# furiosa-ai/eta-inversion

Hardware: AMD Instinct MI355X
Metric: images/sec SD1.5 512^2 50-step etainv+ptp (higher is better)
Workload: dtype bf16; 1 GPU; etainv+ptp, SD1.5-shaped UNet (seeded synthetic weights), 512x512 (64x64 latents), 50 DDIM steps, 32 image pairs per GPU per step, eta [[0.6, 0], [1, 0.7]], n=10 noise candidates, cfg 7.5/1; images_per_gpu=32, unet_sample_forwards_per_image_reference=300

## Files before the change

eta-inversion_amd/csrc/engine.cpp:

```cpp
#include <cmath>
#include <cstring>
#include <functional>
#include <memory>
#include <string>
#include <unordered_map>
#include <vector>

#include "common.h"
#include "kernels.h"

namespace etainv {

static thread_local std::string g_err;
void set_error(const std::string& msg) { g_err = msg; }

struct ProfRec { int cls; double work, bytes; hipEvent_t a, b; };
static bool g_prof_on = false;
static std::vector<ProfRec> g_prof;
static std::vector<std::pair<hipEvent_t, hipEvent_t>> g_prof_pool;
static size_t g_prof_used = 0;
static bool g_prof_paused = false;
bool prof_enabled() { return g_prof_on && !g_prof_paused; }
void prof_pause(bool on) { g_prof_paused = on; }
void prof_begin(int cls, double work, hipStream_t s, double bytes) {
// ... 1380 lines not shown
  p.W = wd;
  p.Ho = upsample ? h * 2 : (stride == 2 ? h / 2 : h);
  p.Wo = upsample ? wd * 2 : (stride == 2 ? wd / 2 : wd);
  p.stride = stride;
  p.ups = upsample;
  p.taps = taps;
  p.M = b * p.Ho * p.Wo;
  p.N = cout;
  p.rows_per_batch = p.Ho * p.Wo;
  return launch_igemm(p, dtype, (hipStream_t)stream);
}

extern "C" int etainv_op_gemm_f32out(const void* a, const void* w, const float* bias, float* out_f32, int m, int n, int k, int dtype, void* stream) {
  IGemmParams p;
  p.a1 = a;
  p.w = w;
  p.bias = bias;
  p.out = out_f32;
  p.out_f32 = 1;
  p.M = m;
  p.N = n;
  p.c1 = k;
  p.W = m;
  p.Wo = m;
  p.rows_per_batch = m;
  return launch_igemm(p, dtype, (hipStream_t)stream);
}

extern "C" int etainv_op_gn_fold(const float* w, const float* gamma, const float* beta, const float* bias, const float* stats, int groups, int b, int n,
                                 int k, void* wb_out, float* cb_out, int dtype, void* stream) {
  return launch_gn_fold(w, gamma, beta, bias, stats, groups, b, n, k, wb_out, cb_out, dtype, (hipStream_t)stream);
}

extern "C" int etainv_op_gemm_per_image(const void* a, const void* wb, const float* cb, const void* residual, void* out, int b, int hw, int n, int k,
                                        int dtype, void* stream) {
  ETAINV_CHECK(b > 0 && hw > 0, "bad sizes");
  IGemmParams p;
  p.a1 = a;
  p.w = wb;
  p.bias = cb;
  p.residual = residual;
  p.out = out;
  p.M = b * hw;
  p.N = n;
  p.c1 = k;
  p.W = p.M;
  p.Wo = p.M;
  p.rows_per_batch = hw;
  p.w_batch_stride = (int64_t)n * k;
  p.bias_batch_stride = n;
  return launch_igemm(p, dtype, (hipStream_t)stream);
}

extern "C" int etainv_op_time_embedding(const int64_t* t_host, int rows, int dim, void* out, int dtype, int via_device, float* t_dev, void* stream) {
  if (!via_device) return launch_time_embedding(t_host, rows, dim, out, dtype, (hipStream_t)stream);
  ETAINV_CHECK(t_dev, "via_device needs t_dev");
  if (launch_set_timesteps(t_host, rows, t_dev, (hipStream_t)stream)) return 1;
  return launch_time_embedding_dev(t_dev, rows, dim, out, dtype, (hipStream_t)stream);
}

extern "C" int etainv_op_silu(const void* x, void* out, int64_t n, int dtype, void* stream) {
  ETAINV_CHECK(x && out && n >= 0, "null pointer or negative size");
  if (n == 0) return 0;
  return launch_silu(x, out, n, dtype, (hipStream_t)stream);
}

extern "C" int etainv_op_cast(const void* src, int src_dtype, void* dst, int dst_dtype, int64_t n, void* stream) {
  ETAINV_CHECK(src && dst && n >= 0, "null pointer or negative size");
  if (n == 0) return 0;
  return launch_cast_f32(src, src_dtype, dst, dst_dtype, n, (hipStream_t)stream);
}

extern "C" int etainv_op_im2col_in(const void* latent, int io_dtype, int n_lat, int rows, int l, void* out, int dtype, void* stream) {
  ETAINV_CHECK(l > 0, "bad sizes");
  return launch_im2col_in(latent, io_dtype, n_lat, rows, l, out, dtype, (hipStream_t)stream);
}

extern "C" int etainv_op_pack_weight(const float* src, void* dst, int64_t rows, int64_t cols, int mode, int taps, float scale, const float* colscale,
                                     int dtype, void* stream) {
  return launch_pack_weight(src, dst, rows, cols, mode, taps, dtype, (hipStream_t)stream, scale, colscale);
}

extern "C" int etainv_op_word_maps_ex(const float* maps_acc, int n_layers, int n_img_cap, int heads, int res, int L, int n_img, const int32_t* tokens,
                                      int n_tok, int steps_done, int row_sel, unsigned layer_mask, float* out, int accumulate, float scale, void* stream) {
  ETAINV_CHECK(row_sel == 0 || row_sel == 1, "row_sel: 0 = source cond row, 1 = target cond row");
  ETAINV_CHECK(n_img <= n_img_cap && heads > 0 && res > 0 && L > 0, "bad sizes");
  return launch_word_maps(maps_acc, n_layers, n_img_cap, 2, row_sel, heads, res, L, n_img, tokens, n_tok, steps_done, out, accumulate, scale,
                          (hipStream_t)stream, layer_mask);
}

extern "C" int etainv_op_word_maps(const float* maps_acc, int n_layers, int n_img_cap, int heads, int res, int L, int n_img,
                                   const int32_t* tokens, int n_tok, int steps_done, float* out, int accumulate, float scale,
                                   void* stream) {
  return launch_word_maps(maps_acc, n_layers, n_img_cap, 2, 0, heads, res, L, n_img, tokens, n_tok, steps_done, out, accumulate, scale,
                          (hipStream_t)stream);
}

extern "C" int etainv_op_local_blend(const float* maps_acc, int n_layers, int n_img_cap, int heads, int res, int L, float* x, int n_img,
                                     const float* blend_alpha, float thres, void* stream) {
  return launch_local_blend(maps_acc, n_layers, n_img_cap, heads, res, L, x, n_img, blend_alpha, thres, (hipStream_t)stream);
}
```

eta-inversion_amd/csrc/igemm.hip:

```cpp
#include <cstdio>
#include <cstdlib>
#include <vector>
#include <type_traits>

#include "common.h"
#include "kernels.h"

namespace etainv {

template <typename T> struct Mfma;
template <> struct Mfma<f16> {
  typedef f16x8 frag;
  static __device__ __forceinline__ f32x4 run(frag a, frag b, f32x4 c) { return __builtin_amdgcn_mfma_f32_16x16x32_f16(a, b, c, 0, 0, 0); }
};
template <> struct Mfma<bf16> {
  typedef bf16x8 frag;
  static __device__ __forceinline__ f32x4 run(frag a, frag b, f32x4 c) { return __builtin_amdgcn_mfma_f32_16x16x32_bf16(a, b, c, 0, 0, 0); }
};

constexpr int BK = 64;
constexpr int64_t SPLITK_WS_BYTES = 64ll << 20;


__device__ __forceinline__ void chan_merge_equal(float n, float& mean, float& m2, float mb, float m2b) {
// ... 1141 lines not shown
  return 0;
#endif
  p.xcd_gn = STAGES == 3 ? pick_xcd_gn(p, BM, BN, grid, tiles) : 1;
  ProfScope prof(PROF_IGEMM, 2.0 * (double)p.M * (double)p.N * (double)(p.taps * (p.c1 + p.c2)), s, igemm_algo_bytes(p));
  hipLaunchKernelGGL((igemm_kernel<T, BM, BN, WAVES_M, STAGES, UPS, LN, PATCH>), dim3(grid), dim3(WAVES_M * 128), lds, s, p);
  ETAINV_LAUNCH_CHECK();
  return 0;
}

template <typename T>
__global__ void __launch_bounds__(256) splitk_reduce_kernel(IGemmParams p) {
  const int n4 = p.N >> 2;
  const int64_t total = (int64_t)p.M * n4;
  for (int64_t idx = (int64_t)blockIdx.x * 256 + threadIdx.x; idx < total; idx += (int64_t)gridDim.x * 256) {
    const int m = (int)(idx / n4), n = (int)(idx - (int64_t)m * n4) * 4;
    f32x4 v = *reinterpret_cast<const f32x4*>(p.ws + (int64_t)m * p.N + n);
    for (int k = 1; k < p.ksplit; ++k) v += *reinterpret_cast<const f32x4*>(p.ws + ((int64_t)k * p.M + m) * p.N + n);
    if (p.ln_stat) {
      v = (v - p.ln_stat[(int64_t)m * 2] * *reinterpret_cast<const f32x4*>(p.ln_s + n)) * p.ln_stat[(int64_t)m * 2 + 1];
    }
    if (p.bias) v += *reinterpret_cast<const f32x4*>(p.bias + (int64_t)(m / p.rows_per_batch) * p.bias_batch_stride + n);
    if (p.rowvec) v += *reinterpret_cast<const f32x4*>(p.rowvec + (int64_t)(m / p.rows_per_batch) * p.rowvec_stride + n);
    if (p.residual) {
      const T* r = reinterpret_cast<const T*>(p.residual) + (int64_t)m * p.N + n;
      v[0] += to_f32(r[0]); v[1] += to_f32(r[1]); v[2] += to_f32(r[2]); v[3] += to_f32(r[3]);
    }
    T o[4] = {from_f32<T>(v[0]), from_f32<T>(v[1]), from_f32<T>(v[2]), from_f32<T>(v[3])};
    *reinterpret_cast<u32x2*>(reinterpret_cast<T*>(p.out) + (int64_t)m * p.N + n) = *reinterpret_cast<u32x2*>(o);
  }
}

static int ring_min_tiles() {
  static const int v = env_int("ETAINV_RING_MIN_TILES", 144);
  return v;
}
static bool ring_fills(const IGemmParams& p) { return (int64_t)cdiv(p.M, 256) * cdiv(p.N, 160) >= ring_min_tiles() && !env_on("ETAINV_NO_RING"); }
static bool ln_ring_ok(const IGemmParams& p) { return !p.ln_stat || p.rows_per_batch % 64 == 0; }

bool igemm_ups4_ok(const IGemmParams& p, int dtype) {
  if (dtype == ETAINV_F32 || p.taps != 4 || p.stride != 1 || p.a2 || p.geglu || p.residual || p.rowvec || p.ln_stat || p.out_f32 || p.out_nchw || p.w_batch_stride || p.pad0) return false;
  if (p.N % 160 != 0 || p.Ho != 2 * p.H || p.Wo != 2 * p.W || p.M % (4 * p.H * p.W) != 0 || p.rows_per_batch != 4 * p.H * p.W) return false;
  if ((p.H * p.W) % 256 != 0 && ((p.M >> 2) % 256 != 0 || (p.H * p.W) % 64 != 0 || !env_flag("ETAINV_UPS4_PM", true))) return false;
  if (p.stat_out && p.stat_kind != 1) return false;
  return env_flag("ETAINV_UPS4", true) && ring_fills(p);
}

bool igemm_hm_ok(const IGemmParams& p, int dtype) {
  if (dtype == ETAINV_F32 || !p.hm_heads || !p.ln_stat || p.geglu || p.taps != 1 || p.a2 || p.residual || p.stat_out || p.out_f32 || p.out_nchw || p.w_batch_stride) return false;
  if ((p.hm_dim != 40 && p.hm_dim != 80) || p.hm_heads != 8 || p.hm_tokens > 16384 || p.M >= (1 << 24)) return false;
  if (p.N != 3 * p.hm_heads * p.hm_dim || p.N % 160 != 0 || p.hm_tokens % 256 != 0 || p.M % p.hm_tokens != 0 || !ln_ring_ok(p)) return false;
  return ring_fills(p);
}

enum IGemmRoute { ROUTE_PPCONV, ROUTE_DUALN, ROUTE_RING_UPS4, ROUTE_RING_UPS9, ROUTE_RING_PATCH, ROUTE_RING, ROUTE_RING_GEGLU, ROUTE_TWO_SLOT };
static const char* const kIGemmRouteName[] = {"ppconv", "dualn", "ring-ups4", "ring-ups9", "ring-patch", "ring", "ring-geglu", "two-slot"};

static IGemmRoute igemm_route(const IGemmParams& p, int dtype) {
  if (pp_conv_applicable(p, dtype)) return ROUTE_PPCONV;
  if (pp_dualn_applicable(p, dtype)) return ROUTE_DUALN;
  if (!p.geglu && p.ups == 2) return ROUTE_RING_UPS4;
  if (!p.geglu && p.ups == 1 && p.N % 160 == 0 && ring_fills(p)) return ROUTE_RING_UPS9;
  if (!p.geglu && p.taps == 9 && p.stride == 1 && !p.ups && !p.a2 && !p.pad0 && p.H % 16 == 0 && p.W % 16 == 0 && p.H == p.Ho && p.W == p.Wo &&
      p.N % 160 == 0 && !p.ln_stat && !p.out_nchw && !p.out_f32 && !p.w_batch_stride && (!p.stat_out || p.stat_kind == 1) &&
      env_flag("ETAINV_PATCHCONV", true) && ring_fills(p))
    return ROUTE_RING_PATCH;
  if (!p.geglu && !p.ups && p.N % 160 == 0 && ring_fills(p) && ln_ring_ok(p)) return ROUTE_RING;
  if (p.geglu && ln_ring_ok(p) && p.c1 >= env_int("ETAINV_GEGLU_RING_MINK", 320) && (int64_t)cdiv(p.M, 256) * cdiv(p.N, 128) >= 256 && !env_on("ETAINV_NO_RING"))
    return ROUTE_RING_GEGLU;
  return ROUTE_TWO_SLOT;
}

static int launch_two_slot(const IGemmParams& p, int dtype, hipStream_t s, int* stat_P) {
  const int64_t big_tiles = (int64_t)cdiv(p.M, 128) * cdiv(p.N, 128);
  static const int deepk_min_tiles = env_int("ETAINV_DEEPK_MIN_TILES", 64);
  static const int deepk_min_nk = env_int("ETAINV_DEEPK_MIN_NK", 64);
  const bool deep_k = !p.geglu && p.N % 160 == 0 && p.taps * (p.c1 + p.c2) / BK >= deepk_min_nk && !p.out_nchw && !p.out_f32 &&
                      (int64_t)cdiv(p.M, 128) * cdiv(p.N, 160) >= deepk_min_tiles;
  const bool big = p.geglu || (big_tiles >= 192 && p.N > 64) || deep_k;
  const int cfg = (big && !p.geglu && p.N % 160 == 0) ? 0 : big ? 1 : 2;
  const int bm = cfg == 2 ? 64 : 128, bn = cfg == 0 ? 160 : cfg == 1 ? 128 : 64;
  const int slots = cfg == 2 ? 1024 : 512;
  const int64_t tiles = (int64_t)cdiv(p.M, bm) * cdiv(p.N, bn);
  const int nk = p.taps * (p.c1 + p.c2) / BK;
  int ks = 1;
  if (!p.geglu && !p.out_nchw && !p.out_f32 && tiles * 2 <= slots && nk >= 16 && !env_on("ETAINV_NO_SPLITK")) {
    static const int max_split = env_int("ETAINV_SPLITK_MAX", 32);
    for (int d = 2; d <= max_split; ++d)
      if (nk % d == 0 && nk / d >= 4 && tiles * d <= slots && (int64_t)p.M * p.N * d * 4 <= SPLITK_WS_BYTES) ks = d;
  }
  static const bool trace = env_on("ETAINV_TRACE_IGEMM");
  if (trace) fprintf(stderr, "  two-slot tile=%dx%d ksplit=%d\n", bm, bn, ks);
  IGemmParams pk = p;
  if (ks > 1) {
    static float* ws[kMaxDevices] = {};
    const int dev = current_device();
    if (!ws[dev]) ETAINV_HIP(hipMalloc(&ws[dev], SPLITK_WS_BYTES));
    pk.ksplit = ks;
    pk.ws = ws[dev];
    pk.bias = nullptr;
    pk.rowvec = nullptr;
    pk.residual = nullptr;
    pk.ln_stat = nullptr;
    pk.stat_out = nullptr;
  }
  ProfScope prof(PROF_IGEMM, 2.0 * (double)p.M * (double)p.N * (double)(p.taps * (p.c1 + p.c2)), s, igemm_algo_bytes(p));
  prof_pause(true);
  int rc = 0;
  ETAINV_DISPATCH_HALF(dtype, T, rc = cfg == 0   ? launch_igemm_t<T, 128, 160, 2, 2, 0, 0>(pk, s, stat_P)
                                      : cfg == 1 ? launch_igemm_t<T, 128, 128, 2, 2, 0, 0>(pk, s, stat_P)
                                                 : launch_igemm_t<T, 64, 64, 2, 2, 0, 0>(pk, s, stat_P));
  prof_pause(false);
// ... 2 lines not shown
    IGemmParams pr = p;
    pr.ksplit = ks;
    pr.ws = pk.ws;
    const int64_t total = (int64_t)p.M * (p.N >> 2);
    ETAINV_DISPATCH_HALF(dtype, T, hipLaunchKernelGGL(splitk_reduce_kernel<T>, dim3((unsigned)std::min<int64_t>(cdiv(total, 256), 2048)),
                                                      dim3(256), 0, s, pr));
    ETAINV_LAUNCH_CHECK();
  }
  return 0;
}

int launch_igemm(const IGemmParams& p_in, int dtype, hipStream_t s, int* stat_P) {
  if (stat_P) *stat_P = 0;
  if (dtype == ETAINV_F32) return launch_igemm_f32(p_in, s);
  static void* zero_pages[kMaxDevices] = {};
  const int dev = current_device();
  if (!zero_pages[dev]) {
    ETAINV_HIP(hipMalloc(&zero_pages[dev], 256));
    ETAINV_HIP(hipMemset(zero_pages[dev], 0, 256));
  }
  IGemmParams p = p_in;
  p.zeros = zero_pages[dev];
  p.debug = env_int("ETAINV_IGEMM_DEBUG", p.debug);
  ETAINV_CHECK(p.a1 && p.w && p.out, "null pointer");
  ETAINV_CHECK(p.M > 0 && p.N > 0 && (p.N % 4) == 0, "N must be a positive multiple of 4");
  ETAINV_CHECK(p.c1 % BK == 0 && p.c2 % BK == 0 && (p.c1 + p.c2) > 0, "channel counts must be multiples of 64");
  ETAINV_CHECK(p.taps == 1 || p.taps == 9 || (p.taps == 4 && p.ups == 2), "taps must be 1 or 9 (4: the phase form of a fused-upsample conv, ups == 2)");
  ETAINV_CHECK(p.taps != 1 || (p.stride == 1 && !p.ups), "1x1 / Linear: stride 1, no upsample");
  ETAINV_CHECK(p.ups != 2 || igemm_ups4_ok(p, dtype), "phase form of the fused-upsample conv: not available for this launch (ask igemm_ups4_ok first)");
  ETAINV_CHECK(!p.geglu || (p.N % 128) == 0, "GEGLU needs N % 128 == 0");
  ETAINV_CHECK(p.rows_per_batch > 0, "rows_per_batch");
  ETAINV_CHECK(!p.rowvec || p.rowvec_stride >= p.N, "rowvec_stride");
  ETAINV_CHECK(!p.ln_stat || (p.ln_s && p.bias && p.taps == 1 && !p.a2), "folded LayerNorm: s / c vectors, plain GEMM");
  ETAINV_CHECK(!p.ln_stat || (!p.residual && !p.rowvec && !p.stat_out), "folded LayerNorm: no residual / row vector / statistics output on the consumer");
  ETAINV_CHECK(!p.ln_stat || (!p.out_f32 && !p.out_nchw), "folded LayerNorm: the consumer stores the compute dtype, row-major (the fp32 / NCHW epilogues do not apply mean / rstd)");
  ETAINV_CHECK(!p.hm_heads || igemm_hm_ok(p, dtype), "head-major QKV output: not available for this launch (ask igemm_hm_ok first)");
  ETAINV_CHECK(!p.out_nchw || p.N == 4, "out_nchw needs N == 4");
  if (p.hm_heads) p.hm_magic = (int)(((1ull << 38) + (unsigned)p.hm_tokens - 1) / (unsigned)p.hm_tokens);
  const IGemmRoute route = igemm_route(p, dtype);
  static const bool trace = env_on("ETAINV_TRACE_IGEMM");
  if (trace)
    fprintf(stderr, "igemm M=%d N=%d c1=%d c2=%d taps=%d stride=%d ups=%d H=%d W=%d geglu=%d ln=%d stat=%d res=%d rowvec=%d hm=%d route=%s\n", p.M, p.N, p.c1, p.c2, p.taps,
            p.stride, p.ups, p.H, p.W, (int)p.geglu, p.ln_stat ? 1 : 0, p.stat_out ? p.stat_kind : 0, p.residual ? 1 : 0, p.rowvec ? 1 : 0, p.hm_heads,
            kIGemmRouteName[route]);
  switch (route) {
    case ROUTE_PPCONV: {
      ProfScope prof(PROF_IGEMM, 2.0 * (double)p.M * (double)p.N * (double)(9 * p.c1), s, igemm_algo_bytes(p));
      return launch_pp_conv(p, dtype, s, stat_P);
    }
    case ROUTE_DUALN: {
      ProfScope prof(PROF_IGEMM, 2.0 * (double)p.M * (double)p.N * (double)(p.c1 + p.c2), s, igemm_algo_bytes(p));
      return launch_pp_dualn(p, dtype, s, stat_P);
    }
    case ROUTE_RING_UPS4:
      p.ups_pm = (p.H * p.W) % 256 != 0;
      ETAINV_DISPATCH_HALF(dtype, T, return (launch_igemm_t<T, 256, 160, 4, 3, 2, 0>(p, s, stat_P)));
      break;
    case ROUTE_RING_UPS9: ETAINV_DISPATCH_HALF(dtype, T, return (launch_igemm_t<T, 256, 160, 4, 3, 1, 0>(p, s, stat_P))); break;
    case ROUTE_RING_PATCH: ETAINV_DISPATCH_HALF(dtype, T, return (launch_igemm_t<T, 256, 160, 4, 3, 0, 0, true>(p, s, stat_P))); break;
    case ROUTE_RING: ETAINV_DISPATCH_HALF(dtype, T, return (launch_igemm_t<T, 256, 160, 4, 3, 0, 0>(p, s, stat_P))); break;
    case ROUTE_RING_GEGLU: ETAINV_DISPATCH_HALF(dtype, T, return (launch_igemm_t<T, 256, 128, 4, 3, 0, 0>(p, s, stat_P))); break;
    case ROUTE_TWO_SLOT: return launch_two_slot(p, dtype, s, stat_P);
  }
  return 0;
}

}
```

eta-inversion_amd/csrc/kernels.h:

```cpp
#pragma once
#include "common.h"

namespace etainv {

struct IGemmParams {
  const void* a1 = nullptr;
  const void* a2 = nullptr;
  const void* w = nullptr;
  const float* bias = nullptr;
  const float* rowvec = nullptr;
  int rowvec_stride = 0;
  int out_f32 = 0;
  int out_nchw = 0;
  int pad0 = 0;
  int out_io_dtype = 0;
  const void* residual = nullptr;
  void* out = nullptr;
  const void* zeros = nullptr;
  int debug = 0;
  int hm_heads = 0, hm_dim = 0, hm_tokens = 0, hm_magic = 0;
  unsigned long* stamps = nullptr;
  int M = 0, N = 0;
  int c1 = 0, c2 = 0;
  int H = 1, W = 1;
  int Ho = 1, Wo = 1;
  int stride = 1, ups = 0, taps = 1;
  int ups_pm = 0;
  int geglu = 0;
  int xcd_gn = 1;
  int ksplit = 1;
  float* ws = nullptr;
  int rows_per_batch = 1;
  int64_t w_batch_stride = 0;
  int bias_batch_stride = 0;
  float* stat_out = nullptr;
  int stat_P = 0;
  int stat_kind = 0;
  const float* ln_stat = nullptr;
  const float* ln_s = nullptr;
};
int launch_igemm(const IGemmParams& p, int dtype, hipStream_t s, int* stat_P = nullptr);
bool igemm_hm_ok(const IGemmParams& p, int dtype);
bool igemm_ups4_ok(const IGemmParams& p, int dtype);

bool pp_dualn_applicable(const IGemmParams& p, int dtype);
bool pp_dualn_hm_ok(const IGemmParams& p, int dtype);
int launch_pp_dualn(const IGemmParams& p, int dtype, hipStream_t s, int* stat_P = nullptr);

bool pp_conv_applicable(const IGemmParams& p, int dtype);
int launch_pp_conv(const IGemmParams& p, int dtype, hipStream_t s, int* stat_P = nullptr);

int launch_igemm_f32(const IGemmParams& p, hipStream_t s);
int launch_groupnorm_f32(const void* x1, const void* x2, int c1, int c2, const float* gamma, const float* beta, void* out, int b, int hw, int groups,
                         float eps, int silu, float* scratch, hipStream_t s);
int launch_layernorm_f32(const void* x, const float* gamma, const float* beta, void* out, int rows, int c, float eps, hipStream_t s);
int launch_self_attention_f32(const void* qkv, void* out, int b, int n, int heads, int d, int mode, int n_img, hipStream_t s, int first_row = 0);
struct CrossParams;
int launch_cross_attention_f32(const void* q, const void* kv, void* out, int b, int d, const CrossParams& p, hipStream_t s);

constexpr int GN_MAX_CHUNKS = 64;
int launch_groupnorm(const void* x1, const void* x2, int c1, int c2, const float* gamma, const float* beta, void* out,
                     int b, int hw, int groups, float eps, int silu, float* scratch, int dtype, hipStream_t s);
int launch_groupnorm_pre(const void* x1, const void* x2, int c1, int c2, const float* part1, int wm1, const float* part2, int wm2, const float* gamma,
                         const float* beta, void* out, int b, int hw, int groups, float eps, int silu, float* final_stats, int dtype, hipStream_t s);
int launch_gn_finalize(int c1, int c2, const float* part1, int wm1, const float* part2, int wm2, int b, int hw, int groups, float eps, float* final_stats,
                       hipStream_t s, const float* gamma = nullptr, const float* beta = nullptr, float* scsh = nullptr);
int launch_gn_fold(const float* w, const float* gamma, const float* beta, const float* bias, const float* final_stats, int groups, int b, int n, int k,
                   void* wb_out, float* cb_out, int dtype, hipStream_t s);
int launch_layernorm(const void* x, const float* gamma, const float* beta, void* out, int rows, int c, float eps, int dtype,
                     hipStream_t s);
int launch_row_stats(const void* x, float* stat, int rows, int c, float eps, int dtype, hipStream_t s);
int launch_ln_finalize(const float* partials, int P, int cw, float eps, float* stat, int rows, hipStream_t s);

inline bool self_attn_prescaled_hm_ok(int d, int dtype) { return dtype != ETAINV_F32 && (d == 40 || d == 80); }
int launch_self_attention_mode(const void* qkv, void* out, int b, int n, int heads, int d, int mode, int n_img, int dtype,
                               hipStream_t s, int q_prescaled = 0, int first_row = 0, int head_major = 0);
struct CrossParams {
  int N = 0, heads = 8, n_ctx = 77;
  float scale_log2 = 0.f;
  int layout = 0;
  int n_img = 1;
  int rows = 0;
  int first_row = 0;
  int edit = 0;
  int map_layer = -1;
  int n_img_cap = 1;
  const int32_t* mapper = nullptr;
  const float* alphas = nullptr;
  const float* replace_mat = nullptr;
  const float* equalizer = nullptr;
  const float* cross_alpha = nullptr;
  float* maps_acc = nullptr;
  int xcd_gx = 0;
};
int launch_cross_attention_p(const void* q, const void* kv, void* out, int b, int d, const CrossParams& p, int dtype, hipStream_t s);

int launch_im2col_in(const void* latent, int io_dtype, int n_lat, int rows, int L, void* out, int dtype, hipStream_t s);
int launch_time_embedding(const int64_t* t_host, int rows, int dim, void* out, int dtype, hipStream_t s);
int launch_set_timesteps(const int64_t* t_host, int rows, float* t_dev, hipStream_t s);
int launch_time_embedding_dev(const float* t_dev, int rows, int dim, void* out, int dtype, hipStream_t s);
// ... 16 lines not shown
```

eta-inversion_amd/etainv/_capi.py:

```python
import ctypes as C
import os
from pathlib import Path

F32, F16, BF16 = 0, 1, 2
ATTN_PLAIN, ATTN_STORE, ATTN_PTP, ATTN_MASA = 0, 1, 2, 3

_LIB_PATH = Path(__file__).resolve().parent / "lib" / "libetainv_hip.so"


class EtainvError(RuntimeError):
    pass


class EngineConfig(C.Structure):
    _fields_ = [("compute_dtype", C.c_int), ("max_unet_batch", C.c_int), ("latent_size", C.c_int), ("max_img", C.c_int),
                ("reserved", C.c_int * 4)]


class AttnCtrl(C.Structure):
    _fields_ = [("mode", C.c_int), ("n_img", C.c_int), ("store_maps", C.c_int),
                ("mapper", C.c_void_p), ("alphas", C.c_void_p), ("replace_mat", C.c_void_p), ("equalizer", C.c_void_p),
                ("cross_alpha", C.c_void_p),
                ("self_replace_active", C.c_int), ("self_max_tokens", C.c_int),
                ("masa_active", C.c_int), ("masa_first_block", C.c_int), ("first_row", C.c_int), ("src_exit_block", C.c_int), ("reserved", C.c_int * 2)]
# ... 22 lines not shown
    "etainv_unet_forward": [_p, _p, _i, C.POINTER(_i64), _p, _i, C.POINTER(AttnCtrl), _p, _i, _p],
    "etainv_maps_reset": [_p, _p],
    "etainv_maps_word_maps": [_p, _i, _p, _i, _i, _p, _i, _f, _p],
    "etainv_maps_word_maps_role": [_p, _i, _p, _i, _i, _i, _p, _i, _f, _p],
    "etainv_maps_configure": [_p, _i, _p],
    "etainv_maps_word_maps_ex": [_p, _i, _p, _i, _i, _i, C.c_uint, _p, _i, _f, _p],
    "etainv_local_blend": [_p, _p, _i, _p, _f, _p],
    "etainv_engine_graph_stats": [_p, C.POINTER(_i64), C.POINTER(_i64)],
    "etainv_engine_qkv_head_major_count": [_p, C.POINTER(C.c_longlong)],
    "etainv_engine_workspace_bytes": [_p],
    "etainv_engine_weight_bytes": [_p],
    "etainv_prof_enable": [_i],
    "etainv_prof_reset": [],
    "etainv_prof_read": [_i, C.POINTER(C.c_double), C.POINTER(C.c_double), C.POINTER(_i64)],
    "etainv_prof_records": [_i, C.POINTER(C.c_double), C.POINTER(C.c_double), _i64, C.POINTER(_i64)],
    "etainv_prof_records_ex": [_i, C.POINTER(C.c_double), C.POINTER(C.c_double), C.POINTER(C.c_double), _i64, C.POINTER(_i64)],
    "etainv_prof_split": [_i, C.c_double, C.POINTER(C.c_double), C.POINTER(_i64)],
    "etainv_op_gemm": [_p, _p, _p, _p, _p, _i, _i, _i, _i, _i, _p],
    "etainv_op_gemm_ln": [_p, _p, _p, _p, _p, _p, _p, _p, C.POINTER(_i), _i, _i, _i, _i, _i, _p],
    "etainv_op_gemm_ln_hm": [_p, _p, _p, _p, _p, _p, _i, _i, _i, _i, _i, _i, C.POINTER(_i), _i, _p],
    "etainv_engine_cache_context": [_p, _i],
    "etainv_engine_context_generation": [_p, C.c_uint64],
    "etainv_op_gemm_gnstat": [_p, _p, _p, _p, _p, _p, C.POINTER(_i), _i, _i, _i, _i, _i, _p],
    "etainv_op_conv3x3_gnstat": [_p, _p, _p, _p, _p, _p, _p, C.POINTER(_i), _i, _i, _i, _i, _i, _i, _p],
    "etainv_op_groupnorm_pre": [_p, _p, _i, _i, _p, _i, _p, _i, _p, _p, _p, _i, _i, _i, _f, _i, _p, _i, _p],
    "etainv_op_ln_fold": [_p, _p, _p, _p, _i, _i, _i, _f, _p, _p, _p, _i, _p],
    "etainv_op_row_stats": [_p, _p, _i, _i, _f, _i, _p],
    "etainv_op_ln_finalize": [_p, _i, _i, _f, _p, _i, _p],
    "etainv_op_pack_ups4": [_p, _p, _i, _i, _i, _p],
    "etainv_op_conv3x3": [_p, _p, _i, _i, _p, _p, _p, _p, _p, _i, _i, _i, _i, _i, _i, _i, _i, _p],
    "etainv_op_conv3x3_ex": [_p, _p, _p, _p, _p, _i, _i, _i, _i, _i, _i, _i, _i, _i, _i, _i, _p],
    "etainv_op_im2col3x3": [_p, _i, _i, _i, _i, _i, _p, _p, _i, _p],
    "etainv_op_row_softmax": [_p, _i, _i, _f, _i, _p],
    "etainv_op_quick_gelu": [_p, _p, _i64, _i, _p],
    "etainv_op_embed": [_p, _p, _p, _i, _i, _i, _p, _i, _p],
    "etainv_op_causal_attention": [_p, _p, _i, _i, _i, _i, _i, _p],
    "etainv_op_groupnorm": [_p, _p, _i, _i, _p, _p, _p, _i, _i, _i, _f, _i, _p, _i, _p],
    "etainv_op_layernorm": [_p, _p, _p, _p, _i, _i, _f, _i, _p],
    "etainv_op_self_attention": [_p, _p, _i, _i, _i, _i, _i, _i, _i, _p],
    "etainv_op_self_attention_ex": [_p, _p, _i, _i, _i, _i, _i, _i, _i, _i, _i, _i, _p],
    "etainv_op_cross_attention": [_p, _p, _p, _i, _i, _i, _i, _i, C.POINTER(AttnCtrl), _i, _i, _p, _i, _p],
    "etainv_op_word_maps": [_p, _i, _i, _i, _i, _i, _i, _p, _i, _i, _p, _i, _f, _p],
    "etainv_op_local_blend": [_p, _i, _i, _i, _i, _i, _p, _i, _p, _f, _p],
    "etainv_op_word_maps_ex": [_p, _i, _i, _i, _i, _i, _i, _p, _i, _i, _i, C.c_uint, _p, _i, _f, _p],
    "etainv_op_time_embedding": [C.POINTER(_i64), _i, _i, _p, _i, _i, _p, _p],
    "etainv_op_silu": [_p, _p, _i64, _i, _p],
    "etainv_op_cast": [_p, _i, _p, _i, _i64, _p],
    "etainv_op_im2col_in": [_p, _i, _i, _i, _i, _p, _i, _p],
    "etainv_op_pack_weight": [_p, _p, _i64, _i64, _i, _i, _f, _p, _i, _p],
    "etainv_op_gemm_f32out": [_p, _p, _p, _p, _i, _i, _i, _i, _p],
    "etainv_op_conv3x3_rv": [_p, _p, _i, _i, _p, _p, _p, _i, _p, _p, _i, _i, _i, _i, _i, _i, _i, _i, _p],
    "etainv_op_gn_fold": [_p, _p, _p, _p, _p, _i, _i, _i, _i, _p, _p, _i, _p],
    "etainv_op_gemm_per_image": [_p, _p, _p, _p, _p, _i, _i, _i, _i, _i, _p],
}
_RESTYPES = {"etainv_last_error": C.c_char_p, "etainv_engine_workspace_bytes": _i64, "etainv_engine_weight_bytes": _i64}

_lib = None


def lib_path() -> Path:
    return Path(os.environ.get("ETAINV_LIB", _LIB_PATH))


def load():
    global _lib
    if _lib is None:
        path = lib_path()
        if not path.exists():
            raise EtainvError(f"{path} not found: build it with eta-inversion_amd/csrc/build.sh (no CPU fallback exists)")
        lib = C.CDLL(str(path))
        for name, args in SIGNATURES.items():
            fn = getattr(lib, name)
            fn.argtypes = args
            fn.restype = _RESTYPES.get(name, C.c_int)
        _lib = lib
    return _lib


def check(status: int):
    if status != 0:
        raise EtainvError(load().etainv_last_error().decode())


def dtype_code(dt) -> int:
    import torch
    return {torch.float32: F32, torch.float16: F16, torch.bfloat16: BF16}[dt]


def ptr(t):
    if t is None:
        return None
    assert t.is_cuda and t.is_contiguous(), "etainv needs contiguous device tensors"
    return t.data_ptr()


def stream_ptr():
    import torch
    return torch.cuda.current_stream().cuda_stream
```

include/etainv.h:

```cpp
#ifndef ETAINV_H
#define ETAINV_H
#include <stdint.h>
#ifdef __cplusplus
extern "C" {
#endif

#define ETAINV_ABI_VERSION 1
#define ETAINV_MAX_WORDS 77

enum etainv_dtype { ETAINV_F32 = 0, ETAINV_F16 = 1, ETAINV_BF16 = 2 };

int etainv_abi_version(void);
const char* etainv_last_error(void);


int etainv_cfg_combine(const void* eps_u, const void* eps_c, float g, void* out, int64_t n,
                       int io_dtype, void* stream);

int etainv_ddim_step(const void* x, const void* eps, float a_from, float a_to, void* out, int64_t n,
                     int io_dtype, void* stream);

int etainv_ddim_eta_step(const void* x, const void* eps, float eta, const void* eta_mask, int n_mask, const void* noise,
                         float a_t, float a_p, float var, int rows, int c, int hw, void* out, int io_dtype, void* stream);

// ... 101 lines not shown
                             float* part, int* wm_out, int b, int h, int wd, int cin, int cout, int dtype, void* stream);
int etainv_op_groupnorm_pre(const void* x1, const void* x2, int c1, int c2, const float* part1, int wm1, const float* part2, int wm2,
                            const float* gamma, const float* beta, void* out, int b, int hw, int groups, float eps, int silu,
                            float* final_stats, int dtype, void* stream);
int etainv_op_pack_ups4(const float* w_oc33, void* dst, int cout, int cin, int dtype, void* stream);
int etainv_op_conv3x3(const void* x_nhwc, const void* x2_nhwc, int c1, int c2, const void* w_okkc, const void* bias,
                      const float* rowvec, const void* residual, void* out, int b, int h, int wd, int cout,
                      int stride, int upsample, int taps, int dtype, void* stream);
int etainv_op_conv3x3_ex(const void* x_nhwc, const void* w_okkc, const void* bias, const void* residual, void* out, int b, int h,
                         int wd, int cin, int cout, int stride, int upsample, int pad0, int out_nchw, int out_io_dtype, int dtype,
                         void* stream);
int etainv_op_im2col3x3(const void* x_nchw, int io_dtype, int cin, int h, int w, int rows, const float* premix, void* out,
                        int dtype, void* stream);
int etainv_op_row_softmax(void* x, int rows, int n, float scale, int dtype, void* stream);
int etainv_op_quick_gelu(const void* x, void* out, int64_t n, int dtype, void* stream);
int etainv_op_embed(const int64_t* ids, const void* tok, const void* pos, int b, int n_pos, int d, void* out, int dtype,
                    void* stream);
int etainv_op_causal_attention(const void* qkv, void* out, int b, int n, int heads, int d, int dtype, void* stream);
int etainv_op_groupnorm(const void* x_nhwc, const void* x2_nhwc, int c1, int c2, const float* gamma,
                        const float* beta, void* out, int b, int hw, int groups, float eps, int silu,
                        float* scratch, int dtype, void* stream);
int etainv_op_layernorm(const void* x, const float* gamma, const float* beta, void* out, int rows, int c,
                        float eps, int dtype, void* stream);
int etainv_op_self_attention(const void* qkv, void* out, int b, int n, int heads, int d, int mode, int n_img,
                             int dtype, void* stream);
int etainv_op_self_attention_ex(const void* qkv, void* out, int b, int n, int heads, int d, int mode, int n_img,
                                int q_prescaled, int first_row, int head_major, int dtype, void* stream);
int etainv_op_cross_attention(const void* q, const void* kv, void* out, int b, int n, int heads, int d,
                              int n_ctx, const etainv_attn_ctrl* ctrl, int map_layer, int n_img_cap,
                              float* maps_acc, int dtype, void* stream);
int etainv_op_word_maps(const float* maps_acc, int n_layers, int n_img_cap, int heads, int res, int L, int n_img,
                        const int32_t* tokens, int n_tok, int steps_done, float* out, int accumulate, float scale,
                        void* stream);
int etainv_op_local_blend(const float* maps_acc, int n_layers, int n_img_cap, int heads, int res, int L, float* x,
                          int n_img, const float* blend_alpha, float thres, void* stream);

int etainv_op_word_maps_ex(const float* maps_acc, int n_layers, int n_img_cap, int heads, int res, int L, int n_img,
                           const int32_t* tokens, int n_tok, int steps_done, int row_sel, unsigned layer_mask, float* out,
                           int accumulate, float scale, void* stream);
int etainv_op_time_embedding(const int64_t* t_host, int rows, int dim, void* out, int dtype, int via_device, float* t_dev, void* stream);
int etainv_op_silu(const void* x, void* out, int64_t n, int dtype, void* stream);
int etainv_op_cast(const void* src, int src_dtype, void* dst, int dst_dtype, int64_t n, void* stream);
int etainv_op_im2col_in(const void* latent, int io_dtype, int n_lat, int rows, int l, void* out, int dtype, void* stream);
int etainv_op_pack_weight(const float* src, void* dst, int64_t rows, int64_t cols, int mode, int taps, float scale, const float* colscale,
                          int dtype, void* stream);
int etainv_op_gemm_f32out(const void* a, const void* w, const float* bias, float* out_f32, int m, int n, int k, int dtype, void* stream);
int etainv_op_conv3x3_rv(const void* x_nhwc, const void* x2_nhwc, int c1, int c2, const void* w_okkc, const void* bias,
                         const float* rowvec, int rowvec_stride, const void* residual, void* out, int b, int h, int wd, int cout,
                         int stride, int upsample, int taps, int dtype, void* stream);
int etainv_op_gn_fold(const float* w, const float* gamma, const float* beta, const float* bias, const float* stats, int groups, int b, int n,
                      int k, void* wb_out, float* cb_out, int dtype, void* stream);
int etainv_op_gemm_per_image(const void* a, const void* wb, const float* cb, const void* residual, void* out, int b, int hw, int n, int k,
                             int dtype, void* stream);

#ifdef __cplusplus
}
#endif
#endif
```

Baseline: 5.716 images/s.

## Add persistent weight-stationary GEMM kernel for 320x320 pointwise projections

Adds a dedicated persistent kernel for 1x1 GEMMs with N=K=320 and large M. Each block keeps the whole 320-column weight slice in registers and streams 64-row activation tiles through a three-deep LDS ring using global-to-LDS DMA. Residual and LN-stat prefetch overlap with the matrix math, and bias, residual, LayerNorm-consumer and row-statistics epilogues are fused. It is routed ahead of the existing ring paths when at least 8192 tiles are present, so it affects the 64x64-resolution projections. The cost is very high register pressure at one block per CU, plus another code path to maintain.

After: 5.736 images/s (median of 6 runs). About the same (+0.4%).

```diff
diff --git a/eta-inversion_amd/csrc/engine.cpp b/eta-inversion_amd/csrc/engine.cpp
--- a/eta-inversion_amd/csrc/engine.cpp
+++ b/eta-inversion_amd/csrc/engine.cpp
@@ -1456,6 +1456,26 @@
   return launch_igemm(p, dtype, (hipStream_t)stream);
 }
 
+extern "C" int etainv_op_gemm_ws320_ok(int m, int n, int k, int k2, int taps, int geglu, int head_major, int out_f32, int out_nchw, int per_image, int rowvec,
+                                       int dtype) {
+  static const float one = 1.0f;
+  IGemmParams p;
+  p.M = m;
+  p.N = n;
+  p.c1 = k;
+  p.c2 = k2;
+  if (k2) p.a2 = &one;
+  p.taps = taps;
+  p.geglu = geglu;
+  if (head_major) { p.hm_heads = 8; p.hm_dim = 40; p.hm_tokens = 256; }
+  p.out_f32 = out_f32;
+  p.out_nchw = out_nchw ? 4 : 0;
+  if (per_image) { p.w_batch_stride = (int64_t)n * k; p.bias_batch_stride = n; }
+  if (rowvec) { p.rowvec = &one; p.rowvec_stride = n; }
+  p.rows_per_batch = m;
+  return ws320_applicable(p, dtype) ? 1 : 0;
+}
+
 extern "C" int etainv_op_time_embedding(const int64_t* t_host, int rows, int dim, void* out, int dtype, int via_device, float* t_dev, void* stream) {
   if (!via_device) return launch_time_embedding(t_host, rows, dim, out, dtype, (hipStream_t)stream);
   ETAINV_CHECK(t_dev, "via_device needs t_dev");
diff --git a/eta-inversion_amd/csrc/igemm.hip b/eta-inversion_amd/csrc/igemm.hip
--- a/eta-inversion_amd/csrc/igemm.hip
+++ b/eta-inversion_amd/csrc/igemm.hip
@@ -1217,11 +1217,12 @@
   return ring_fills(p);
 }
 
-enum IGemmRoute { ROUTE_PPCONV, ROUTE_DUALN, ROUTE_RING_UPS4, ROUTE_RING_UPS9, ROUTE_RING_PATCH, ROUTE_RING, ROUTE_RING_GEGLU, ROUTE_TWO_SLOT };
-static const char* const kIGemmRouteName[] = {"ppconv", "dualn", "ring-ups4", "ring-ups9", "ring-patch", "ring", "ring-geglu", "two-slot"};
+enum IGemmRoute { ROUTE_PPCONV, ROUTE_DUALN, ROUTE_RING_UPS4, ROUTE_RING_UPS9, ROUTE_RING_PATCH, ROUTE_RING, ROUTE_RING_GEGLU, ROUTE_TWO_SLOT, ROUTE_WS320 };
+static const char* const kIGemmRouteName[] = {"ppconv", "dualn", "ring-ups4", "ring-ups9", "ring-patch", "ring", "ring-geglu", "two-slot", "ws320"};
 
 static IGemmRoute igemm_route(const IGemmParams& p, int dtype) {
   if (pp_conv_applicable(p, dtype)) return ROUTE_PPCONV;
+  if (ws320_applicable(p, dtype)) return ROUTE_WS320;
   if (pp_dualn_applicable(p, dtype)) return ROUTE_DUALN;
   if (!p.geglu && p.ups == 2) return ROUTE_RING_UPS4;
   if (!p.geglu && p.ups == 1 && p.N % 160 == 0 && ring_fills(p)) return ROUTE_RING_UPS9;
@@ -1330,6 +1331,10 @@
       ProfScope prof(PROF_IGEMM, 2.0 * (double)p.M * (double)p.N * (double)(p.c1 + p.c2), s, igemm_algo_bytes(p));
       return launch_pp_dualn(p, dtype, s, stat_P);
     }
+    case ROUTE_WS320: {
+      ProfScope prof(PROF_IGEMM, 2.0 * (double)p.M * (double)p.N * (double)p.c1, s, igemm_algo_bytes(p));
+      return launch_ws320(p, dtype, s, stat_P);
+    }
     case ROUTE_RING_UPS4:
       p.ups_pm = (p.H * p.W) % 256 != 0;
       ETAINV_DISPATCH_HALF(dtype, T, return (launch_igemm_t<T, 256, 160, 4, 3, 2, 0>(p, s, stat_P)));
diff --git a/eta-inversion_amd/csrc/kernels.h b/eta-inversion_amd/csrc/kernels.h
--- a/eta-inversion_amd/csrc/kernels.h
+++ b/eta-inversion_amd/csrc/kernels.h
@@ -46,6 +46,9 @@
 bool pp_dualn_applicable(const IGemmParams& p, int dtype);
 bool pp_dualn_hm_ok(const IGemmParams& p, int dtype);
 int launch_pp_dualn(const IGemmParams& p, int dtype, hipStream_t s, int* stat_P = nullptr);
+
+bool ws320_applicable(const IGemmParams& p, int dtype);
+int launch_ws320(const IGemmParams& p, int dtype, hipStream_t s, int* stat_P = nullptr);
 
 bool pp_conv_applicable(const IGemmParams& p, int dtype);
 int launch_pp_conv(const IGemmParams& p, int dtype, hipStream_t s, int* stat_P = nullptr);
diff --git a/eta-inversion_amd/csrc/wsgemm.hip b/eta-inversion_amd/csrc/wsgemm.hip
--- /dev/null
+++ b/eta-inversion_amd/csrc/wsgemm.hip
@@ -0,0 +1,354 @@
+#include <algorithm>
+#include <cstdio>
+#include <cstdlib>
+#include <type_traits>
+
+#include "common.h"
+#include "kernels.h"
+
+namespace etainv {
+
+namespace {
+
+template <typename T> struct WMfma;
+template <> struct WMfma<f16> {
+  typedef f16x8 frag;
+  static __device__ __forceinline__ f32x4 run(frag a, frag b, f32x4 c) { return __builtin_amdgcn_mfma_f32_16x16x32_f16(a, b, c, 0, 0, 0); }
+};
+template <> struct WMfma<bf16> {
+  typedef bf16x8 frag;
+  static __device__ __forceinline__ f32x4 run(frag a, frag b, f32x4 c) { return __builtin_amdgcn_mfma_f32_16x16x32_bf16(a, b, c, 0, 0, 0); }
+};
+
+#define WS_VMCNT(n) __builtin_amdgcn_s_waitcnt(0x0F70 | ((n) & 15) | (((n) >> 4) << 14))
+#define WS_DMA(voff32, sbase, ldsaddr) \
+  asm volatile("s_mov_b32 m0, %2\n\ts_nop 0\n\tglobal_load_lds_dwordx4 %0, %1" : : "v"(voff32), "s"(sbase), "s"(__builtin_amdgcn_readfirstlane(ldsaddr)) : "memory")
+
+constexpr int WC = 320;
+constexpr int WBM = 64;
+constexpr int WKT = WC / 64;
+constexpr int WNT = 5, WMT = 4;
+constexpr int WKT_BYTES = WBM * 64 * 2;
+constexpr int WTILE_BYTES = WKT * WKT_BYTES;
+constexpr int WRING = 3;
+constexpr int WLDS = WRING * WTILE_BYTES;
+constexpr int WPIECES = 2 * WKT;
+
+__device__ __forceinline__ float ws_row_sum16(float x) {
+  x += __builtin_bit_cast(float, __builtin_amdgcn_update_dpp(0, __builtin_bit_cast(int, x), 0xB1, 0xf, 0xf, true));
+  x += __builtin_bit_cast(float, __builtin_amdgcn_update_dpp(0, __builtin_bit_cast(int, x), 0x4E, 0xf, 0xf, true));
+  x += __builtin_bit_cast(float, __builtin_amdgcn_update_dpp(0, __builtin_bit_cast(int, x), 0x141, 0xf, 0xf, true));
+  x += __builtin_bit_cast(float, __builtin_amdgcn_update_dpp(0, __builtin_bit_cast(int, x), 0x140, 0xf, 0xf, true));
+  return x;
+}
+
+template <typename T, int EPI, bool RES, int STAT>
+__global__ void __launch_bounds__(256, 1) ws320_kernel(IGemmParams p) {
+  typedef typename WMfma<T>::frag frag;
+  constexpr bool LNC = EPI == 1;
+  static_assert(!LNC || (!RES && !STAT), "a LayerNorm consumer has no residual and emits no statistics");
+  constexpr int N = WC;
+  constexpr int NPF = (RES ? WMT * WNT : 0) + (LNC ? WMT : 0);
+  constexpr int NBEHIND = WPIECES + 2 * (NPF + 3 * WMT);
+  constexpr int NWAIT = NBEHIND < 63 ? NBEHIND : 63;
+  extern __shared__ __attribute__((aligned(16))) char smem[];
+
+  const int tid = threadIdx.x, lane = tid & 63;
+  const int wid = __builtin_amdgcn_readfirstlane(tid >> 6);
+  const int fr = lane & 15, fq = lane >> 4;
+  const int tiles = p.M / WBM;
+  const int G = gridDim.x;
+  const int my_tiles = (tiles - (int)blockIdx.x + G - 1) / G;
+  if (my_tiles <= 0) return;
+  auto tile_m0 = [&](int i) __attribute__((always_inline)) { return ((int)blockIdx.x + (i < my_tiles ? i : my_tiles - 1) * G) * WBM; };
+  const bool has_bias = p.bias != nullptr;
+
+  T* const out = reinterpret_cast<T*>(p.out);
+  const T* const res = reinterpret_cast<const T*>(p.residual);
+  const int col0 = wid * 80;
+  const int lane_col = col0 + fq * 4;
+
+  u32x2 rvA[WMT][WNT] = {}, rvB[WMT][WNT] = {};
+  f32x2 stA[WMT], stB[WMT];
+#pragma unroll
+  for (int i = 0; i < WMT; ++i) stA[i] = stB[i] = (f32x2){0.f, 1.f};
+  auto prefetch = [&](int m0, auto& r, auto& s2) __attribute__((always_inline)) {
+    if constexpr (RES) {
+      const T* rb = res + (int64_t)(m0 + fr) * N + lane_col;
+#pragma unroll
+      for (int i = 0; i < WMT; ++i)
+#pragma unroll
+        for (int j = 0; j < WNT; ++j) r[i][j] = *reinterpret_cast<const u32x2*>(rb + i * 16 * N + j * 16);
+    }
+    if constexpr (LNC) {
+#pragma unroll
+      for (int i = 0; i < WMT; ++i) s2[i] = *reinterpret_cast<const f32x2*>(p.ln_stat + (int64_t)(m0 + i * 16 + fr) * 2);
+    }
+  };
+  prefetch(tile_m0(0), rvA, stA);
+
+  u32x4 wf[2 * WKT][WNT];
+  {
+    const char* wb = reinterpret_cast<const char*>(p.w) + ((col0 + fr) * WC + fq * 8) * 2;
+#pragma unroll
+    for (int ks = 0; ks < 2 * WKT; ++ks)
+#pragma unroll
+      for (int j = 0; j < WNT; ++j) wf[ks][j] = *reinterpret_cast<const u32x4*>(wb + j * (16 * WC * 2) + ks * 64);
+#pragma unroll
+    for (int ks = 0; ks < 2 * WKT; ++ks)
+#pragma unroll
+      for (int j = 0; j < WNT; ++j) asm volatile("" : "+a"(wf[ks][j]));
+  }
+  f32x4 bv[WNT], sv[WNT];
+#pragma unroll
+  for (int j = 0; j < WNT; ++j) {
+    bv[j] = has_bias ? *reinterpret_cast<const f32x4*>(p.bias + lane_col + j * 16) : (f32x4){0.f, 0.f, 0.f, 0.f};
+    sv[j] = (f32x4){0.f, 0.f, 0.f, 0.f};
+    if constexpr (LNC) sv[j] = *reinterpret_cast<const f32x4*>(p.ln_s + lane_col + j * 16);
+  }
+
+  const unsigned lrow = tid >> 3;
+  unsigned voff[2];
+#pragma unroll
+  for (int h = 0; h < 2; ++h) voff[h] = ((lrow + 32 * h) * (unsigned)WC + (((tid & 7) ^ (lrow & 7)) << 3)) * 2u;
+  const unsigned lds0 = (unsigned)(unsigned long long)(__attribute__((address_space(3))) char*)smem;
+  auto issue_tile = [&](int i) __attribute__((always_inline)) {
+    const char* g = reinterpret_cast<const char*>(p.a1) + (int64_t)tile_m0(i) * (WC * 2);
+    const unsigned d = lds0 + (unsigned)(i % WRING) * WTILE_BYTES + wid * 1024;
+#pragma unroll
+    for (int kt = 0; kt < WKT; ++kt) {
+      WS_DMA(voff[0], g + kt * 128, d + kt * WKT_BYTES);
+      WS_DMA(voff[1], g + kt * 128, d + kt * WKT_BYTES + 4096);
+    }
+  };
+
+  unsigned a_rd[2];
+#pragma unroll
+  for (int kk = 0; kk < 2; ++kk) a_rd[kk] = (fr * 64 + (((kk * 4 + fq) ^ (fr & 7)) << 3)) * 2;
+  f32x4 acc[WMT][WNT];
+
+  auto epilogue = [&](int m0, auto& rv, auto& st) __attribute__((always_inline)) {
+    const int mrow = m0 + fr;
+    const int64_t lane_off = (int64_t)mrow * N + col0;
+    if constexpr (STAT == 2) {
+      const int64_t rt = m0 / 64;
+      float* gs = p.stat_out;
+      auto do_pair = [&](auto j0_tag, auto nb_tag) __attribute__((always_inline)) {
+        constexpr int j0 = decltype(j0_tag)::value, NB = decltype(nb_tag)::value;
+        f32x4 sm[NB], sq[NB];
+#pragma unroll
+        for (int jj = 0; jj < NB; ++jj) sm[jj] = sq[jj] = (f32x4){0.f, 0.f, 0.f, 0.f};
+#pragma unroll
+        for (int i = 0; i < WMT; ++i) {
+          u32x2 po[NB];
+#pragma unroll
+          for (int jj = 0; jj < NB; ++jj) {
+            f32x4 v = acc[i][j0 + jj];
+            if (has_bias) v += bv[j0 + jj];
+            if constexpr (RES) {
+              T r[4];
+              *reinterpret_cast<u32x2*>(r) = rv[i][j0 + jj];
+              v[0] += to_f32(r[0]); v[1] += to_f32(r[1]); v[2] += to_f32(r[2]); v[3] += to_f32(r[3]);
+            }
+            T o[4] = {from_f32<T>(v[0]), from_f32<T>(v[1]), from_f32<T>(v[2]), from_f32<T>(v[3])};
+            po[jj] = *reinterpret_cast<u32x2*>(o);
+#pragma unroll
+            for (int q = 0; q < 4; ++q) {
+              const float x = to_f32(o[q]);
+              sm[jj][q] += x;
+              sq[jj][q] += x * x;
+            }
+          }
+          T* prow = out + lane_off + (int64_t)i * 16 * N;
+          if constexpr (NB == 2) {
+            const auto lo = __builtin_amdgcn_permlane16_swap(po[0][0], po[1][0], false, false);
+            const auto hi = __builtin_amdgcn_permlane16_swap(po[0][1], po[1][1], false, false);
+            const u32x4 v = {lo[0], hi[0], lo[1], hi[1]};
+            *reinterpret_cast<u32x4*>(prow + (j0 + (fq & 1)) * 16 + (fq >> 1) * 8) = v;
+          } else {
+            *reinterpret_cast<u32x2*>(prow + j0 * 16 + fq * 4) = po[0];
+          }
+        }
+#pragma unroll
+        for (int jj = 0; jj < NB; ++jj) {
+#pragma unroll
+          for (int q = 0; q < 4; ++q) {
+            sm[jj][q] = ws_row_sum16(sm[jj][q]);
+            sq[jj][q] = ws_row_sum16(sq[jj][q]);
+          }
+          const int n = col0 + (j0 + jj) * 16 + fq * 4;
+          if (fr == 0) {
+            *reinterpret_cast<f32x4*>(gs + (rt * 2 + 0) * N + n) = sm[jj];
+            *reinterpret_cast<f32x4*>(gs + (rt * 2 + 1) * N + n) = sq[jj];
+          }
+        }
+      };
+      do_pair(std::integral_constant<int, 0>{}, std::integral_constant<int, 2>{});
+      do_pair(std::integral_constant<int, 2>{}, std::integral_constant<int, 2>{});
+      do_pair(std::integral_constant<int, 4>{}, std::integral_constant<int, 1>{});
+    } else {
+#pragma unroll
+      for (int i = 0; i < WMT; ++i) {
+        u32x2 po[WNT];
+#pragma unroll
+        for (int j = 0; j < WNT; ++j) {
+          f32x4 v = acc[i][j];
+          if constexpr (LNC) {
+            v = (v - st[i][0] * sv[j]) * st[i][1] + bv[j];
+          } else {
+            if (has_bias) v += bv[j];
+          }
+          if constexpr (RES) {
+            T r[4];
+            *reinterpret_cast<u32x2*>(r) = rv[i][j];
+            v[0] += to_f32(r[0]); v[1] += to_f32(r[1]); v[2] += to_f32(r[2]); v[3] += to_f32(r[3]);
+          }
+          T o[4] = {from_f32<T>(v[0]), from_f32<T>(v[1]), from_f32<T>(v[2]), from_f32<T>(v[3])};
+          po[j] = *reinterpret_cast<u32x2*>(o);
+        }
+        T* prow = out + lane_off + (int64_t)i * 16 * N;
+#pragma unroll
+        for (int k = 0; k + 1 < WNT; k += 2) {
+          const auto lo = __builtin_amdgcn_permlane16_swap(po[k][0], po[k + 1][0], false, false);
+          const auto hi = __builtin_amdgcn_permlane16_swap(po[k][1], po[k + 1][1], false, false);
+          const u32x4 v = {lo[0], hi[0], lo[1], hi[1]};
+          *reinterpret_cast<u32x4*>(prow + (k + (fq & 1)) * 16 + (fq >> 1) * 8) = v;
+        }
+        *reinterpret_cast<u32x2*>(prow + (WNT - 1) * 16 + fq * 4) = po[WNT - 1];
+        if constexpr (STAT == 1) {
+          float sum = 0.f;
+#pragma unroll
+          for (int j = 0; j < WNT; ++j) {
+            T o[4];
+            *reinterpret_cast<u32x2*>(o) = po[j];
+            sum += (to_f32(o[0]) + to_f32(o[1])) + (to_f32(o[2]) + to_f32(o[3]));
+          }
+          float mu = sum * (1.0f / (float)(WNT * 4)), m2 = 0.f;
+#pragma unroll
+          for (int j = 0; j < WNT; ++j) {
+            T o[4];
+            *reinterpret_cast<u32x2*>(o) = po[j];
+#pragma unroll
+            for (int q = 0; q < 4; ++q) { const float d = to_f32(o[q]) - mu; m2 += d * d; }
+          }
+          {
+            const float mo = __shfl_xor(mu, 16, 64), qo = __shfl_xor(m2, 16, 64);
+            const bool odd = fq & 1;
+            float ma = odd ? mo : mu, mb = odd ? mu : mo, qa = odd ? qo : m2, qb = odd ? m2 : qo;
+            float d = mb - ma;
+            ma += 0.5f * d;
+            qa += qb + d * d * (0.5f * (float)(WNT * 4));
+            const float mo2 = __shfl_xor(ma, 32, 64), qo2 = __shfl_xor(qa, 32, 64);
+            const bool hi = fq >> 1;
+            float m_lo = hi ? mo2 : ma, m_hi = hi ? ma : mo2, q_lo = hi ? qo2 : qa, q_hi = hi ? qa : qo2;
+            d = m_hi - m_lo;
+            mu = m_lo + 0.5f * d;
+            m2 = q_lo;
+            m2 += q_hi + d * d * (0.5f * (float)(2 * WNT * 4));
+          }
+          if (fq == 0) *reinterpret_cast<f32x2*>(p.stat_out + ((int64_t)(mrow + i * 16) * p.stat_P + wid) * 2) = (f32x2){mu, m2};
+        }
+      }
+    }
+  };
+
+  issue_tile(0);
+  if (my_tiles > 1) issue_tile(1);
+
+  auto tile_step = [&](int t, auto& rv, auto& st, auto& rvn, auto& stn) __attribute__((always_inline)) {
+    __builtin_amdgcn_sched_barrier(0);
+    if (t + 1 < my_tiles) {
+      if (t >= 2) WS_VMCNT(NWAIT); else WS_VMCNT(WPIECES);
+    } else {
+      WS_VMCNT(0);
+    }
+    __builtin_amdgcn_sched_barrier(0);
+    __builtin_amdgcn_s_barrier();
+    __builtin_amdgcn_sched_barrier(0);
+    if (t + 2 < my_tiles) issue_tile(t + 2);
+    __builtin_amdgcn_sched_barrier(0);
+
+    const char* abuf = smem + (t % WRING) * WTILE_BYTES;
+#pragma unroll
+    for (int i = 0; i < WMT; ++i)
+#pragma unroll
+      for (int j = 0; j < WNT; ++j) acc[i][j] = (f32x4){0.f, 0.f, 0.f, 0.f};
+#pragma unroll
+    for (int kt = 0; kt < WKT; ++kt)
+#pragma unroll
+      for (int kk = 0; kk < 2; ++kk) {
+        u32x4 fa[WMT];
+        const char* ba = abuf + kt * WKT_BYTES + a_rd[kk];
+#pragma unroll
+        for (int i = 0; i < WMT; ++i) fa[i] = *reinterpret_cast<const u32x4*>(ba + i * (16 * 64 * 2));
+#pragma unroll
+        for (int i = 0; i < WMT; ++i)
+#pragma unroll
+          for (int j = 0; j < WNT; ++j)
+            acc[i][j] = WMfma<T>::run(__builtin_bit_cast(frag, wf[kt * 2 + kk][j]), __builtin_bit_cast(frag, fa[i]), acc[i][j]);
+      }
+    __builtin_amdgcn_sched_barrier(0);
+    prefetch(tile_m0(t + 1), rvn, stn);
+    __builtin_amdgcn_sched_barrier(0);
+    epilogue(tile_m0(t), rv, st);
+  };
+  for (int t = 0; t < my_tiles; t += 2) {
+    tile_step(t, rvA, stA, rvB, stB);
+    if (t + 1 < my_tiles) tile_step(t + 1, rvB, stB, rvA, stA);
+  }
+}
+
+template <typename T, int EPI, bool RES, int STAT>
+void launch_ws320_t(const IGemmParams& p, int grid, hipStream_t s) {
+  allow_dynamic_lds<&ws320_kernel<T, EPI, RES, STAT>>(WLDS);
+  hipLaunchKernelGGL((ws320_kernel<T, EPI, RES, STAT>), dim3(grid), dim3(256), WLDS, s, p);
+}
+
+}
+
+bool ws320_applicable(const IGemmParams& p, int dtype) {
+  if (!env_flag("ETAINV_WS320", true) || (dtype != ETAINV_F16 && dtype != ETAINV_BF16)) return false;
+  if (p.N != WC || p.c1 != WC || p.a2 || p.c2 || p.taps != 1) return false;
+  if (p.geglu || p.hm_heads || p.out_f32 || p.out_nchw || p.w_batch_stride || p.rowvec || p.ksplit > 1 || p.debug) return false;
+  if (p.M <= 0 || p.M % WBM != 0 || p.M / WBM < std::max(1, env_int("ETAINV_WS320_MIN_TILES", 8192))) return false;
+  if (p.ln_stat && (!p.ln_s || !p.bias || p.residual || p.stat_out)) return false;
+  if (p.stat_out && p.stat_kind == 1 && p.rows_per_batch % WBM != 0) return false;
+  return true;
+}
+
+int launch_ws320(const IGemmParams& p_in, int dtype, hipStream_t s, int* stat_P) {
+  IGemmParams p = p_in;
+  ETAINV_CHECK(ws320_applicable(p, dtype), "not a ws320 launch (ask ws320_applicable first)");
+  if (p.stat_out) p.stat_P = p.stat_kind == 1 ? WBM : WC / 80;
+  if (stat_P) *stat_P = p.stat_out ? p.stat_P : 0;
+  const int tiles = p.M / WBM;
+  int cus = 256;
+  {
+    static int cu_count[kMaxDevices] = {};
+    const int dev = current_device();
+    if (!cu_count[dev]) {
+      int n = 0;
+      if (hipDeviceGetAttribute(&n, hipDeviceAttributeMultiprocessorCount, dev) != hipSuccess || n <= 0) n = 256;
+      cu_count[dev] = n;
+    }
+    cus = cu_count[dev];
+  }
+  const int grid_env = env_int("ETAINV_WS320_GRID", 0);
+  const int grid = std::min(tiles, grid_env ? std::max(1, grid_env) : cus);
+  ETAINV_DISPATCH_HALF(dtype, T, {
+    if (p.ln_stat) launch_ws320_t<T, 1, false, 0>(p, grid, s);
+    else if (p.residual) {
+      if (p.stat_out && p.stat_kind == 1) launch_ws320_t<T, 0, true, 2>(p, grid, s);
+      else if (p.stat_out) launch_ws320_t<T, 0, true, 1>(p, grid, s);
+      else launch_ws320_t<T, 0, true, 0>(p, grid, s);
+    } else {
+      if (p.stat_out && p.stat_kind == 1) launch_ws320_t<T, 0, false, 2>(p, grid, s);
+      else if (p.stat_out) launch_ws320_t<T, 0, false, 1>(p, grid, s);
+      else launch_ws320_t<T, 0, false, 0>(p, grid, s);
+    }
+  });
+  ETAINV_LAUNCH_CHECK();
+  return 0;
+}
+
+}
diff --git a/eta-inversion_amd/etainv/_capi.py b/eta-inversion_amd/etainv/_capi.py
--- a/eta-inversion_amd/etainv/_capi.py
+++ b/eta-inversion_amd/etainv/_capi.py
@@ -98,6 +98,7 @@
     "etainv_op_conv3x3_rv": [_p, _p, _i, _i, _p, _p, _p, _i, _p, _p, _i, _i, _i, _i, _i, _i, _i, _i, _p],
     "etainv_op_gn_fold": [_p, _p, _p, _p, _p, _i, _i, _i, _i, _p, _p, _i, _p],
     "etainv_op_gemm_per_image": [_p, _p, _p, _p, _p, _i, _i, _i, _i, _i, _p],
+    "etainv_op_gemm_ws320_ok": [_i] * 12,
 }
 _RESTYPES = {"etainv_last_error": C.c_char_p, "etainv_engine_workspace_bytes": _i64, "etainv_engine_weight_bytes": _i64}
 
diff --git a/include/etainv.h b/include/etainv.h
--- a/include/etainv.h
+++ b/include/etainv.h
@@ -177,6 +177,8 @@
                       int k, void* wb_out, float* cb_out, int dtype, void* stream);
 int etainv_op_gemm_per_image(const void* a, const void* wb, const float* cb, const void* residual, void* out, int b, int hw, int n, int k,
                              int dtype, void* stream);
+int etainv_op_gemm_ws320_ok(int m, int n, int k, int k2, int taps, int geglu, int head_major, int out_f32, int out_nchw, int per_image, int rowvec,
+                            int dtype);
 
 #ifdef __cplusplus
 }
```
